# mycophonic/saprobe-alac

Measured on AMD Instinct MI355X. Metric: Msamples/s decoded (16-bit stereo, 4096-frame packets), higher is better.
Workload: dtype int32; 1 GPU; 65536 packets/GPU x 16-bit 2-ch 4096-frame ALAC, music-like synthetic, device-resident in/out; packets_per_gpu=65536

## Files before the change

### saprobe-alac_amd/csrc/alac_duo.h

```cpp
#ifndef ALAC_DUO_H
#define ALAC_DUO_H

#include <type_traits>

#include "alac_regular.h"

namespace alac {

constexpr uint32_t DUO_CHUNK = 16;
constexpr int DUO_UN8_MAX = 12;
enum { ROLE_A = 0, ROLE_B = 1, ROLE_BOTH = 2, ROLE_C = 3 };

template <class W, class B, int NA, int OUT, int ROLE, bool F16, bool NARROW, bool EA, bool UN8W = false, bool EC = false, int WMODE = 0>
ALAC_DEV void duo_phase(W& wv, const DevCfg& cfg, const B& bits, RegLane<W>& s, uint32_t size, uint32_t ns,
                        uint32_t n_it, uint32_t hdr_pos, uint32_t den_shift, uint32_t chan_bits, int32_t mix_res,
                        uint32_t mix_sh, uint32_t na_rt, uint32_t shift_pos, uint32_t sb, uint32_t mode) {
    constexpr bool DO_A = ROLE == ROLE_A || ROLE == ROLE_BOTH, DO_B = ROLE == ROLE_B || ROLE == ROLE_BOTH;
    constexpr bool RAW = OUT == OUT_RAW;
    constexpr bool LAST = OUT == OUT_STEREO || OUT == OUT_MONO || RAW;
    constexpr bool CPE = OUT == OUT_STEREO;
    constexpr bool QND = W::kResMem || EC;
    constexpr bool GEN = NA == 0;
    constexpr int NR = GEN ? 1 : NA;
    constexpr bool WRAP = !(NA == 4 || NA == 5 || NA == 6 || NA == 8);
// ... 54 lines not shown
    const uint32_t nzm = mix_res != 0 ? 0xffffffffu : 0u;

    uint32_t ns_live = s.err == 0 ? ns : 0u;
    if (DO_A) gol_head(s, c31kb);
    auto qval = [&](uint32_t nd) -> int32_t { return QND ? (int32_t)nd : gol_unfold(nd); };
    auto golomb_chunk = [&](uint32_t c) {
        const uint32_t buf = c & 1u;
        if ((c + 1u) * CH <= n_it) {
#pragma nounroll
            for (uint32_t g = 0; g < CH; g += GOL_TICK) {
                s.rd.tick(wv, s.pos);
                s.near = gol_near(s, c * CH + g, ns_live);
#pragma nounroll
                for (uint32_t h = g; h < g + GOL_TICK; h += 4u) {
#pragma unroll
                    for (uint32_t j = 0; j < 4u; ++j)
                        wv.rq_write(buf, h + j, qval(gol_step<true>(wv, bits, s, size, kb, wb, c31kb, chan_bits, c * CH + h + j, ns, ns_live)));
                }
            }
            return;
        }
#pragma nounroll
        for (uint32_t j = 0; j < CH; ++j) {
            const uint32_t i = c * CH + j;
            if (i >= n_it) break;
            if ((i & (GOL_TICK - 1u)) == 0) {
                s.rd.tick(wv, s.pos);
                s.near = gol_near(s, i, ns_live);
            }
            wv.rq_write(buf, j, qval(gol_step<true>(wv, bits, s, size, kb, wb, c31kb, chan_bits, i, ns, ns_live)));
        }
    };
    constexpr bool FP_OK = F16 && CPE && LAST && !EMIT_A && !RAW;
    uint32_t fp_base = 0, fp_inc = 0;
    using fp_yes = std::integral_constant<bool, true>;
    using fp_no = std::integral_constant<bool, false>;
    auto emit = [&](uint32_t i, int32_t o, int32_t u, uint64_t sw, uint32_t jj, auto fp) {
        constexpr bool FP = decltype(fp)::value;
        const bool on = i < ns;
        if (RAW) {
            wv.st_push_if((uint32_t)o, on);
            return;
        }
        int32_t l = o, r = 0;
        if (CPE) {
            const int32_t vv = o;
            const int32_t mv = NARROW ? ALAC_MUL24(mix_res, vv) : (int32_t)((uint32_t)mix_res * (uint32_t)vv);
            l = u + (int32_t)((uint32_t)vv & nzm) - (mv >> mix_sh);
            r = (int32_t)((((uint32_t)(l - vv)) & nzm) | ((uint32_t)vv & ~nzm));
        }
        if (F16) {
            const uint32_t pcm = ((uint32_t)l & 0xffffu) | ((uint32_t)r << 16);
            if (FP) wv.st_put(fp_base, jj, pcm, fp_inc);
            else wv.st_push_if(pcm, on);
            return;
        }
        if (cfg.bit_depth == 20) {
            l = (int32_t)((uint32_t)l << 4);
            r = (int32_t)((uint32_t)r << 4);
        }
        if (merge_any) {
            const uint32_t sh_l = sb ? (uint32_t)(sw >> (64u - sb)) : 0u;
            const uint32_t sh_r = (CPE && sb) ? (uint32_t)((sw << sb) >> (64u - sb)) : 0u;
            l = (int32_t)((uint32_t)l << sb) | (int32_t)sh_l;
            r = (int32_t)((uint32_t)r << sb) | (int32_t)sh_r;
        }
// ... 97 lines not shown
    uint64_t sw_n[CH];
    uint32_t g_n[CH / 4u][3] = {};
    auto fetch_mem_ahead = [&](uint32_t c) {
        const bool blocks = whole_pk3(c);
#pragma unroll
        for (uint32_t j = 0; j < CH; ++j) {
            const uint32_t i = c * CH + j;
            u_n[j] = 0;
            sw_n[j] = 0;
            if (i < n_it) {
                if (CPE) u_n[j] = *wv.u_row(i);
                if (merge_any && !blocks) sw_n[j] = bits.window_raw(shift_pos + i * sstep_a);
            }
        }
        if (PK3C && blocks && sb8) {
#pragma unroll
            for (uint32_t q = 0; q < CH / 4u; ++q) bits.load12(sh_byte + 2u * (c * CH + 4u * q), g_n[q][0], g_n[q][1], g_n[q][2]);
        }
    };
    auto emit_chunk = [&](uint32_t c) {
        if (PK3C && whole_pk3(c)) {
#pragma unroll
            for (uint32_t q = 0; q < CH / 4u; ++q) {
                int32_t vv4[4], uu4[4];
#pragma unroll
                for (uint32_t j = 0; j < 4u; ++j) {
                    vv4[j] = sq_v[4u * q + j];
                    uu4[j] = u_v[4u * q + j];
                }
                pk3_block(c * CH + 4u * q, vv4, uu4, g_v[q][0], g_v[q][1], g_v[q][2]);
            }
            return;
        }
#pragma unroll
        for (uint32_t j = 0; j < CH; ++j) {
            const uint32_t i = c * CH + j;
            if (i < n_it) emit(i, sq_v[j], u_v[j], sw_v[j], 0u, fp_no{});
        }
        wv.st_step();
    };
    constexpr uint32_t UN = (NARROW && (((F16 || !LAST || RAW || EMIT_A) && NR <= DUO_UN8_MAX) || (UN8W && NR <= 8))) ? 8u : 4u;
    constexpr bool HBM_IN = LAST && !RAW && !EMIT_A;
    constexpr bool RMEM = W::kResMem && ROLE == ROLE_B;
    int32_t dpre[UN];
    uint32_t dpre_row = 0xffffffffu;
    int32_t upre[UN];
    uint64_t spre[UN];
    uint32_t pre_row = 0xffffffffu;
    constexpr uint32_t NSUB = UN / 4u;
    uint32_t gpre[NSUB][3] = {};
    auto prefetch_group = [&](uint32_t row0) {
        pre_row = row0;
#pragma unroll
        for (uint32_t j = 0; j < UN; ++j) {
            upre[j] = 0;
            spre[j] = 0;
            if (CPE) upre[j] = *wv.u_row(row0 + j);
            if (merge_any && !pk3) spre[j] = bits.window_raw(shift_pos + (row0 + j) * sstep_b);
        }
        if (PK3 && pk3 && sb8) {
#pragma unroll
            for (uint32_t q = 0; q < NSUB; ++q) bits.load12(sh_byte + 2u * (row0 + 4u * q), gpre[q][0], gpre[q][1], gpre[q][2]);
        }
    };
    auto predict_chunk = [&](uint32_t c) {
        const uint32_t buf = c & 1u;
        const bool simple = GEN && (na == 0 || na == 31);
        const uint32_t sstep = (CPE ? 2u : 1u) * sb;
        if (!simple && !mode_any && c * CH > na && (c + 1u) * CH <= n_it) {
            auto groups = [&](auto wrap, auto fp) {
                constexpr bool FP = decltype(fp)::value;
#pragma nounroll
// ... 456 lines not shown
```

### saprobe-alac_amd/csrc/alac_gpu.h

```cpp
#ifndef ALAC_GPU_H
#define ALAC_GPU_H
#include <hip/hip_runtime.h>

#include <algorithm>
#include <cstdio>
#include <cstdlib>
#include <cstring>

#define ALAC_DEV __device__ __forceinline__
#define ALAC_HD __host__ __device__ __forceinline__
#define ALAC_NOINLINE
#define ALAC_MUL24(a, b) __mul24((int)(a), (int)(b))
__device__ __forceinline__ uint32_t alac_sad(uint32_t a, uint32_t b, uint32_t c) {
    uint32_t r;
    asm("v_sad_u32 %0, %1, %2, %3" : "=v"(r) : "v"(a), "v"(b), "v"(c));
    return r;
}
#define ALAC_SAD(a, b, c) alac_sad((uint32_t)(a), (uint32_t)(b), (uint32_t)(c))

__device__ __forceinline__ int32_t alac_sign_med3(int32_t x) {
    int32_t r;
    asm("v_med3_i32 %0, %1, -1, 1" : "=v"(r) : "v"(x));
    return r;
}
// ... 104 lines not shown
#ifndef ALAC_LDS_ROWS
#define ALAC_LDS_ROWS 64
#endif
#ifndef ALAC_LDS_RING
#define ALAC_LDS_RING 32
#endif
#ifndef ALAC_LDS_FLUSH
#define ALAC_LDS_FLUSH (ALAC_LDS_ROWS / 2)
#endif
constexpr uint32_t kRing = ALAC_LDS_ROWS;
constexpr uint32_t kFlush = ALAC_LDS_FLUSH;
static_assert(kFlush <= kRing && kRing % 4 == 0 && (kFlush == 16 || kFlush == 32), "the stager flushes 64- or 128-byte pieces of its rows");
constexpr uint32_t kRowStride = kRing + 1;
constexpr uint32_t kFallbackSlots = 64;
constexpr uint32_t kRingDw = ALAC_LDS_RING;
constexpr uint32_t kRingSlots = kRingDw + 2;

constexpr uint32_t kKeys = alac::KEY_IRREGULAR + 2u;
constexpr uint32_t kKeyLegacy = alac::KEY_IRREGULAR;
constexpr uint32_t kKeyScan = alac::KEY_IRREGULAR + 1u;
struct Plan {
    uint32_t count[kKeys];
    uint32_t pkt_start[kKeys];
    uint32_t cursor[kKeys];
    uint32_t nk;
    uint32_t list_key[kKeys];
    uint32_t list_wave0[kKeys];
    uint32_t total_waves;
    uint32_t irr_waves;
    uint32_t wide_waves;
    uint32_t gate[2][512];
    uint32_t balance[2][512];
    uint32_t queue[2];
};

static __shared__ uint32_t s_rows[kWave * kRowStride];
static __shared__ unsigned long long s_optr[kWave];
static __shared__ __attribute__((aligned(16))) uint32_t s_ring[kRingSlots * kWave];
constexpr uint32_t kQ = alac::DUO_CHUNK;
static __shared__ int32_t s_rq[2 * kQ * kWave];

__host__ __device__ inline size_t u_tile_cells(uint32_t frame_length) { return ((size_t)frame_length + 1u) * kWave; }

struct GpuWave {
    static constexpr bool kResMem = false;
    static constexpr uint32_t kRingDw = alack::kRingDw;
    int32_t* u_tile;
    int32_t* g_tile;
    uint8_t* my_out;
    uint32_t lane, wcnt, flushed;
    uint32_t ppw;

    ALAC_DEV bool any(bool p) const { return __ballot(p) != 0ull; }
    ALAC_DEV uint32_t max_u32(uint32_t v) const {
#pragma unroll
        for (int o = 32; o > 0; o >>= 1) {
            const uint32_t t = (uint32_t)__shfl_xor((int)v, o, 64);
            v = t > v ? t : v;
        }
        return (uint32_t)__builtin_amdgcn_readfirstlane((int)v);
    }
    static constexpr bool kRingPow2 = (kRing & (kRing - 1u)) == 0u;
    uint32_t wpos, fpos;
    ALAC_DEV static uint32_t umin_(uint32_t a, uint32_t b) { return a < b ? a : b; }
    ALAC_DEV static uint32_t st_wrap(uint32_t x) { return kRingPow2 ? (x & (kRing - 1u)) : umin_(x, x - kRing); }
    ALAC_DEV uint32_t st_pos() const { return kRingPow2 ? (wcnt & (kRing - 1u)) : wpos; }
// ... 121 lines not shown
    }
    ALAC_DEV uint32_t quad_from_below(uint32_t x, uint32_t fresh, uint32_t q0m) const {
        return ALAC_BFI(q0m, fresh, (uint32_t)__builtin_amdgcn_mov_dpp((int)x, 0x90, 0xf, 0xf, true));
    }
    ALAC_DEV void duo_sync() { asm volatile("s_waitcnt lgkmcnt(0)\n\ts_barrier" ::: "memory"); }
    ALAC_DEV void duo_sync_mem() {
        __threadfence_block();
        __syncthreads();
    }
    ALAC_DEV int32_t* u_row(uint32_t i) const { return u_tile + ((size_t)i * kWave + (ppw < kWave ? (lane < ppw ? lane : ppw) : lane)); }
    ALAC_DEV int32_t* g_slot(uint32_t k) const { return g_tile + (size_t)k * ppw; }
};

struct GpuWaveMem : GpuWave {
    static constexpr bool kResMem = true;
    const int32_t* res;
    uint32_t it, chunk0;
    ALAC_DEV int32_t rq_read(uint32_t, uint32_t j) const { return res[chunk0 + j]; }
    ALAC_DEV void rq_write(uint32_t, uint32_t, int32_t) {}
    ALAC_DEV void duo_sync() {
        ++it;
        chunk0 = (it - 1u) * kQ;
    }
    ALAC_DEV void duo_sync_mem() {}
};

__device__ __forceinline__ uint32_t avail_of(uint64_t blob_bytes, uint64_t off) {
    const uint64_t left = blob_bytes - off;
    return left > 0xffffffffull ? 0xffffffffu : (uint32_t)left;
}

__global__ void alac_classify(alac::DevCfg cfg, const uint8_t* __restrict__ blob, uint64_t blob_bytes, const uint64_t* __restrict__ offsets,
                              const uint32_t* __restrict__ sizes, uint32_t n, uint16_t* __restrict__ keys, uint32_t* __restrict__ sizes_ws,
                              uint32_t* __restrict__ frames_out, int32_t* __restrict__ status, Plan* plan);
__global__ void alac_plan(Plan* plan, uint32_t ppw);
__global__ void alac_cu_census(uint32_t* __restrict__ seen, uint32_t* __restrict__ arrived, uint32_t expect);
__global__ void alac_scatter(const uint16_t* __restrict__ keys, uint32_t n, Plan* plan, uint32_t* __restrict__ perm);
__global__ void alac_task_classify(alac::DevCfg cfg, const alac::ChanDesc* __restrict__ cd, const alac::PktDesc* __restrict__ pd,
                                   const uint16_t* __restrict__ pkt_keys, uint32_t n_slots, uint16_t* __restrict__ keys, Plan* plan);
__global__ void alac_scan(alac::DevCfg cfg, const uint8_t* __restrict__ blob, uint64_t blob_bytes, const uint64_t* __restrict__ offsets,
                          const uint32_t* __restrict__ sizes, const uint32_t* __restrict__ perm, const Plan* __restrict__ plan,
                          uint8_t* __restrict__ out, uint64_t out_stride, uint32_t* __restrict__ frames_out,
                          int32_t* __restrict__ status, int32_t* __restrict__ scratch_u, int32_t* __restrict__ scratch_g,
                          uint32_t ppw, alac::ChanDesc* __restrict__ cd, alac::PktDesc* __restrict__ pd, int32_t* __restrict__ rows,
                          uint64_t row_stride);
__global__ void alac_legacy(alac::DevCfg cfg, const uint8_t* __restrict__ blob, uint64_t blob_bytes, const uint64_t* __restrict__ offsets,
                            const uint32_t* __restrict__ sizes, const uint32_t* __restrict__ perm, const Plan* __restrict__ plan,
                            const alac::PktDesc* __restrict__ pd, uint8_t* __restrict__ out, uint64_t out_stride,
                            uint32_t* __restrict__ frames_out, int32_t* __restrict__ status, int32_t* __restrict__ scratch_u,
                            int32_t* __restrict__ scratch_g, uint32_t ppw);
constexpr uint32_t kModeFit4 = 4u, kModeFit5 = 5u, kModeGated = 6u;
constexpr __host__ __device__ __forceinline__ uint32_t decode_mode(uint32_t items, uint32_t n_cu, uint32_t cap, uint32_t force, bool mono,
                                                                  bool fit5) {
    if (force == kModeFit4 || (force == kModeFit5 && fit5)) return force;
    if (items <= 4u * n_cu) return kModeFit4;
    if (items <= 5u * n_cu) return (cap >= 5u && !mono) ? kModeGated : fit5 ? kModeFit5 : kModeFit4;
    if (items <= 6u * n_cu && cap >= 6u) return kModeGated;
    return (2u * items <= 15u * n_cu || !fit5) ? kModeFit4 : kModeFit5;
}
constexpr __host__ __device__ __forceinline__ uint32_t pair_quota(uint32_t items, uint32_t n_cu, uint32_t cap) {
    const uint32_t need = (items + n_cu - 1u) / n_cu;
    return need < 5u ? 5u : need < cap ? need : cap;
}
constexpr bool mode_is_fit4_without_the_others(uint32_t n_cu) {
    for (uint32_t items = 0u; items <= 40u * n_cu; items += (items < 8u * n_cu ? 1u : n_cu / 2u + 1u))
        if (decode_mode(items, n_cu, 0u, 0u, false, false) != kModeFit4 || decode_mode(items, n_cu, 0u, 5u, true, false) != kModeFit4) return false;
    return true;
}
constexpr bool mode_is_fit4_within_four(uint32_t n_cu) {
    for (uint32_t cap = 0u; cap <= 8u; ++cap)
// ... 52 lines not shown
```

### saprobe-alac_amd/csrc/alacgpu.hip

```cpp
#include "alac_gpu.h"
#include "alac_host.h"
#include "alac_waveform.h"

using namespace alack;

namespace {
thread_local char g_err[512] = "";
}

void alack::set_err(const char* fmt, ...) {
    va_list ap;
    va_start(ap, fmt);
    vsnprintf(g_err, sizeof(g_err), fmt, ap);
    va_end(ap);
}

namespace {

class CopyPool {
public:
    explicit CopyPool(unsigned threads) {
        for (unsigned t = 0; t < threads; ++t) workers_.emplace_back([this] { run(); });
    }
    ~CopyPool() {
// ... 97 lines not shown
Kernels choose_kernels(const alac::DevCfg& c) {
    Kernels k{};
    k.lean = alac::lean_config(c);
    k.one_or_two = c.num_channels <= 2;
    k.quad = c.bit_depth == 16 ? ALAC_PAIR_KERNEL(alac_decode_16q) : c.bit_depth == 32 ? ALAC_PAIR_KERNEL(alac_decode_32q) : ALAC_PAIR_KERNEL(alac_decode_24q);
    k.gated = c.bit_depth == 16 ? ALAC_PAIR_KERNEL(alac_decode_16g) : PairKernel{nullptr, ""};
    k.wide = c.bit_depth == 32 ? ALAC_PAIR_KERNEL(alac_decode_w32) : c.bit_depth == 24 ? ALAC_PAIR_KERNEL(alac_decode_w24) : PairKernel{nullptr, ""};
    const bool four_frames = c.num_channels > 2 && (c.num_channels * c.bps) % 4u == 0u;
    k.interleave = four_frames ? alac_interleave4 : alac_interleave;
    k.interleave_lds = (four_frames ? 128u : 32u) * kWave;
    k.irregular = !k.lean        ? "alac_scan (whole-packet decoder)"
                  : k.one_or_two ? "alac_scan + alac_interleave (+ alac_legacy)"
                  : four_frames  ? "alac_scan + alac_chan_predict + alac_interleave4 (+ alac_legacy)"
                                 : "alac_scan + alac_chan_predict + alac_interleave (+ alac_legacy)";
    return k;
}
#undef ALAC_PAIR_KERNEL

}

struct alacgpu_decoder {
    alacgpu_config cfg;
    alac::DevCfg dev_cfg;
    Kernels kernels;
    int device;
    size_t frame_bytes;
    hipStream_t stream;
    hipStream_t s_in, s_out;
    hipStream_t s_side;
    hipEvent_t ev_fork, ev_join;
    hipEvent_t ev_start[kTimingSlots], ev_stop[kTimingSlots];
    uint64_t launches;
    DevBuf scratch_u, scratch_g, plan, cls, perm, sizes_ws;
    DevBuf cd, pd, plan2, keys2, perm2, rows;
    Slot slots[kSlots];
    CopyPool* pool;
    uint32_t n_cu;
    DevBuf cu_number;
    size_t chunk_bytes;
    uint32_t lanes_min;
    int side;
    std::thread* ahead;
    int ahead_rc;
    char ahead_err[512];
    size_t last_n;
    uint32_t last_ppw, last_cap, last_fit5;
    uint32_t fit_force;
    DevBuf wave_ws;
    hipEvent_t ev_w0, ev_w1;
    bool wave_timed;
};

namespace {

size_t plan_claims_offset() { return (sizeof(Plan) + 255u) & ~(size_t)255u; }
size_t plan_bytes(size_t waves) { return plan_claims_offset() + waves * 4 * sizeof(uint32_t); }

struct KernelAttr {
    uint32_t pairs_per_cu, static_lds;
};
KernelAttr kernel_attr(void (*kernel)(PairArgs)) {
    static std::mutex mu;
    static std::vector<std::pair<const void*, KernelAttr>> cache;
    std::lock_guard<std::mutex> g(mu);
    for (const auto& e : cache)
        if (e.first == (const void*)kernel) return e.second;
    int v = 0;
    hipFuncAttributes at;
    KernelAttr a{4u, kQuadLdsFit4};
    if (hipOccupancyMaxActiveBlocksPerMultiprocessor(&v, kernel, (int)(2 * kWave), 0) == hipSuccess && v > 0) a.pairs_per_cu = (uint32_t)v;
    else (void)hipGetLastError();
    if (hipFuncGetAttributes(&at, (const void*)kernel) == hipSuccess) a.static_lds = (uint32_t)at.sharedSizeBytes;
    else (void)hipGetLastError();
    cache.emplace_back((const void*)kernel, a);
    return a;
}

int cu_numbers(alacgpu_decoder* dec) {
    int rc;
    if ((rc = dec->cu_number.ensure(513 * sizeof(uint32_t)))) return rc;
    HIP_TRY(hipMemsetAsync(dec->cu_number.p, 0, 513 * sizeof(uint32_t), dec->stream));
    hipLaunchKernelGGL(alac_cu_census, dim3(2 * dec->n_cu), dim3(kWave), 0, dec->stream, (uint32_t*)dec->cu_number.p,
                       (uint32_t*)dec->cu_number.p + 512, 2 * dec->n_cu);
    HIP_TRY(hipGetLastError());
    uint32_t seen[512];
    HIP_TRY(hipMemcpyAsync(seen, dec->cu_number.p, sizeof(seen), hipMemcpyDeviceToHost, dec->stream));
    HIP_TRY(hipStreamSynchronize(dec->stream));
    uint32_t per_xcd[8] = {0}, xcds = 0, total = 0;
    for (uint32_t i = 0; i < 512; i++)
// ... 10 lines not shown
        if (seen[i]) {
            const uint32_t x = i >> 6;
            seen[i] = 1u + next[x]++ * xcds + order[x];
        }
    if (total > dec->n_cu) dec->n_cu = total;
    HIP_TRY(hipMemcpyAsync(dec->cu_number.p, seen, sizeof(seen), hipMemcpyHostToDevice, dec->stream));
    HIP_TRY(hipStreamSynchronize(dec->stream));
    return ALACGPU_E_OK;
}

size_t max_waves(uint32_t bit_depth, size_t n, uint32_t ppw) {
    const size_t keys = (bit_depth >= 24 ? 2 : 1) * 18 * 18 + 8;
    return (n + ppw - 1) / ppw + std::min<size_t>(n, keys);
}
size_t max_waves(const alacgpu_decoder* dec, size_t n, uint32_t ppw) { return max_waves(dec->cfg.bit_depth, n, ppw); }

uint32_t pick_ppw(size_t n) {
    if (const char* e = getenv("ALACGPU_PPW")) {
        const int v = atoi(e);
        if (v >= 1 && v <= 64) return (uint32_t)v;
    }
    uint32_t ppw = kWave;
    while (ppw > 1 && n / ppw < 256) ppw >>= 1;
    return ppw;
}

size_t row_stride_of(uint32_t frame_length) { return ((size_t)frame_length + 3u) & ~(size_t)3u; }

int reserve_workspace(alacgpu_decoder* dec, size_t n, uint32_t ppw) {
    const size_t waves = max_waves(dec, n, ppw);
    int rc;
    if ((rc = dec->scratch_u.ensure(waves * u_tile_cells(dec->cfg.frame_length) * sizeof(int32_t)))) return rc;
    if ((rc = dec->scratch_g.ensure(waves * kFallbackSlots * ppw * sizeof(int32_t)))) return rc;
    if ((rc = dec->plan.ensure(plan_bytes(waves)))) return rc;
    if ((rc = dec->cls.ensure((n ? n : 1) * sizeof(uint16_t)))) return rc;
    if ((rc = dec->perm.ensure((n ? n : 1) * sizeof(uint32_t)))) return rc;
    if ((rc = dec->sizes_ws.ensure((n ? n : 1) * sizeof(uint32_t)))) return rc;
    const size_t ns = (n ? n : 1) * 8;
    if ((rc = dec->cd.ensure(ns * sizeof(alac::ChanDesc)))) return rc;
    if ((rc = dec->pd.ensure((n ? n : 1) * sizeof(alac::PktDesc)))) return rc;
    if (dec->cfg.num_channels > 2) {
        if ((rc = dec->plan2.ensure(sizeof(Plan)))) return rc;
        if ((rc = dec->keys2.ensure(ns * sizeof(uint16_t)))) return rc;
        if ((rc = dec->perm2.ensure(ns * sizeof(uint32_t)))) return rc;
        if ((rc = dec->rows.ensure((n ? n : 1) * dec->cfg.num_channels * row_stride_of(dec->cfg.frame_length) * sizeof(int32_t))))
            return rc;
    }
    return ALACGPU_E_OK;
}

struct Launch {
    alacgpu_decoder* dec;
    alac::DevCfg c;
    const uint8_t* d_blob;
    uint64_t blob_bytes;
    const uint64_t* d_offsets;
    size_t n;
    uint8_t* d_out;
    size_t out_stride;
    uint32_t* d_frames;
    int32_t* d_status;
    uint32_t ppw;
    size_t waves;
    hipStream_t irr;
    bool forked;
    uint32_t scan_grid;
    Plan* plan() const { return (Plan*)dec->plan.p; }
    const uint32_t* sz() const { return (const uint32_t*)dec->sizes_ws.p; }
};

struct SideFork {
    alacgpu_decoder* dec;
    bool open = false;
    int fork() {
        HIP_TRY(hipEventRecord(dec->ev_fork, dec->stream));
        HIP_TRY(hipStreamWaitEvent(dec->s_side, dec->ev_fork, 0));
        open = true;
        return ALACGPU_E_OK;
    }
    int join() {
        HIP_TRY(hipEventRecord(dec->ev_join, dec->s_side));
        HIP_TRY(hipStreamWaitEvent(dec->stream, dec->ev_join, 0));
        open = false;
        return ALACGPU_E_OK;
    }
    ~SideFork() {
        if (open) (void)hipStreamSynchronize(dec->s_side);
    }
};

int sort_pass(const Launch& L, const uint32_t* d_sizes) {
    alacgpu_decoder* dec = L.dec;
    const uint32_t nb = (uint32_t)((L.n + 255) / 256);
    HIP_TRY(hipMemsetAsync(L.plan(), 0, plan_bytes(L.waves), dec->stream));
    hipLaunchKernelGGL(alac_classify, dim3(nb), dim3(256), 0, dec->stream, L.c, L.d_blob, L.blob_bytes, L.d_offsets, d_sizes,
                       (uint32_t)L.n, (uint16_t*)dec->cls.p, (uint32_t*)dec->sizes_ws.p, L.d_frames, L.d_status, L.plan());
    hipLaunchKernelGGL(alac_plan, dim3(1), dim3(kWave), 0, dec->stream, L.plan(), L.ppw);
    hipLaunchKernelGGL(alac_scatter, dim3(nb), dim3(256), 0, dec->stream, (const uint16_t*)dec->cls.p, (uint32_t)L.n, L.plan(),
                       (uint32_t*)dec->perm.p);
    return ALACGPU_E_OK;
}

void scan(const Launch& L) {
    alacgpu_decoder* dec = L.dec;
    hipLaunchKernelGGL(alac_scan, dim3(L.scan_grid), dim3(kWave), 0, L.irr, L.c, L.d_blob, L.blob_bytes,
                       L.d_offsets, L.sz(), (const uint32_t*)dec->perm.p, (const Plan*)L.plan(), L.d_out, (uint64_t)L.out_stride, L.d_frames,
                       L.d_status, (int32_t*)dec->scratch_u.p, (int32_t*)dec->scratch_g.p, L.ppw, (alac::ChanDesc*)dec->cd.p,
                       (alac::PktDesc*)dec->pd.p, dec->cfg.num_channels > 2 ? (int32_t*)dec->rows.p : (int32_t*)nullptr,
                       (uint64_t)row_stride_of(dec->cfg.frame_length));
}

void narrow_launch(const Launch& L, const PairArgs& a, uint32_t slots, uint32_t mode) {
    alacgpu_decoder* dec = L.dec;
    const Kernels& k = dec->kernels;
    if (mode == kModeGated) {
        if (a.cap) hipLaunchKernelGGL(k.gated.fn, dim3(std::min<uint32_t>(a.cap * dec->n_cu, slots)), dim3(2 * kWave), 0, dec->stream, a);
        return;
    }
    if (mode == kModeFit5 && !a.fit5) return;
    const uint32_t stat = kernel_attr(k.quad.fn).static_lds;
    PairArgs q = a;
    q.fit = mode;
    hipLaunchKernelGGL(k.quad.fn, dim3(slots), dim3(4 * kWave), (mode == kModeFit4 && stat < kQuadLdsFit4) ? kQuadLdsFit4 - stat : 0u,
                       dec->stream, q);
}

void regular_packets(const Launch& L) {
    alacgpu_decoder* dec = L.dec;
    const Kernels& k = dec->kernels;
    const size_t n = L.n;
    const uint32_t ppw = L.ppw;
    PairArgs a{L.c, L.d_blob, (uint64_t)L.blob_bytes, L.d_offsets, L.sz(), (const uint32_t*)dec->perm.p, L.plan(), L.d_out, (uint64_t)L.out_stride,
               L.d_frames, L.d_status, (int32_t*)dec->scratch_u.p, (const uint32_t*)dec->cu_number.p,
               (uint32_t*)((uint8_t*)L.plan() + plan_claims_offset()), ppw, dec->n_cu, 0u, dec->lanes_min, 4u, dec->fit_force, 0u};
    const uint32_t slots = (uint32_t)L.waves;
    const uint32_t n_cu = dec->n_cu;
    const bool beyond4 = (n + ppw - 1) / ppw > (size_t)4 * n_cu || dec->fit_force == kModeFit5;
    const bool has_twin = k.gated.fn && beyond4 && dec->fit_force == 0u;
    {
        const uint32_t stat = kernel_attr(k.quad.fn).static_lds;
        a.fit5 = (beyond4 && (size_t)((stat + 1279u) / 1280u) * 1280u * 5u <= 163840u) ? 1u : 0u;
    }
    if (has_twin) a.cap = kernel_attr(k.gated.fn).pairs_per_cu;
    if (a.cap <= 4u) a.cap = 0u;
    dec->last_cap = a.cap;
    dec->last_fit5 = a.fit5;
    const uint32_t guess = decode_mode((uint32_t)((n + ppw - 1) / ppw), n_cu, a.cap, dec->fit_force, dec->cfg.num_channels == 1, a.fit5 != 0u);
    narrow_launch(L, a, slots, guess);
    if (k.wide.fn) hipLaunchKernelGGL(k.wide.fn, dim3(slots), dim3(2 * kWave), 0, dec->stream, a);
    for (uint32_t mode : {kModeFit4, kModeFit5, kModeGated})
        if (mode != guess) narrow_launch(L, a, slots, mode);
}

int split_pipeline(const Launch& L) {
    alacgpu_decoder* dec = L.dec;
    Plan* plan2 = (Plan*)dec->plan2.p;
    const size_t n_slots = L.n * 8;
    const uint32_t nb2 = (uint32_t)((n_slots + 255) / 256);
    const uint32_t ppw2 = pick_ppw(L.n * dec->cfg.num_channels);
    HIP_TRY(hipMemsetAsync(plan2, 0, sizeof(Plan), dec->stream));
    hipLaunchKernelGGL(alac_task_classify, dim3(nb2), dim3(256), 0, dec->stream, L.c, (const alac::ChanDesc*)dec->cd.p,
                       (const alac::PktDesc*)dec->pd.p, (const uint16_t*)dec->cls.p, (uint32_t)n_slots,
                       (uint16_t*)dec->keys2.p, plan2);
    hipLaunchKernelGGL(alac_plan, dim3(1), dim3(kWave), 0, dec->stream, plan2, ppw2);
    hipLaunchKernelGGL(alac_scatter, dim3(nb2), dim3(256), 0, dec->stream, (const uint16_t*)dec->keys2.p,
                       (uint32_t)n_slots, plan2, (uint32_t*)dec->perm2.p);
    hipLaunchKernelGGL(alac_chan_predict, dim3((uint32_t)max_waves(16u, n_slots, ppw2)), dim3(kWave), 0, dec->stream, L.c,
                       L.d_blob, L.blob_bytes, L.d_offsets, L.sz(), (const uint32_t*)dec->perm2.p, (const Plan*)plan2,
                       (const alac::ChanDesc*)dec->cd.p, (int32_t*)dec->rows.p, (uint64_t)row_stride_of(dec->cfg.frame_length), ppw2);
    return ALACGPU_E_OK;
}

void irregular_pcm(const Launch& L) {
    alacgpu_decoder* dec = L.dec;
    const Kernels& k = dec->kernels;
    const uint64_t rs = row_stride_of(dec->cfg.frame_length);
    const uint32_t bpp = (dec->cfg.frame_length + kWave - 1u) / kWave;
    const uint32_t ib = (uint32_t)std::min<uint64_t>((uint64_t)L.n * ((bpp + 7u) / 8u), L.forked ? (uint64_t)4 * dec->n_cu : (uint64_t)32768u);
    hipLaunchKernelGGL(k.interleave, dim3(ib), dim3(kWave), k.interleave_lds, L.irr, L.c, L.d_blob, L.blob_bytes, L.d_offsets, L.sz(),
                       (const uint32_t*)dec->perm.p, (const Plan*)L.plan(), (const alac::ChanDesc*)dec->cd.p,
                       (const alac::PktDesc*)dec->pd.p, (const int32_t*)dec->rows.p, rs, L.d_out, (uint64_t)L.out_stride, bpp);
    hipLaunchKernelGGL(alac_legacy, dim3(L.scan_grid), dim3(kWave), 0, L.irr, L.c, L.d_blob, L.blob_bytes,
                       L.d_offsets, L.sz(), (const uint32_t*)dec->perm.p, (const Plan*)L.plan(), (const alac::PktDesc*)dec->pd.p, L.d_out,
                       (uint64_t)L.out_stride, L.d_frames, L.d_status, (int32_t*)dec->scratch_u.p, (int32_t*)dec->scratch_g.p, L.ppw);
}

int launch(alacgpu_decoder* dec, const uint8_t* d_blob, uint64_t blob_bytes, const uint64_t* d_offsets,
           const uint32_t* d_sizes, size_t n, uint8_t* d_out, size_t out_stride, uint32_t* d_frames, int32_t* d_status) {
    if (n == 0) return ALACGPU_E_OK;
    if (n > 0x7fffffffu) {
        set_err("batch too large");
        return ALACGPU_E_ARG;
    }
    const uint32_t ppw = pick_ppw(n);
    int rc = reserve_workspace(dec, n, ppw);
    if (rc) return rc;
    dec->last_n = n;
    dec->last_ppw = ppw;
    dec->last_cap = dec->last_fit5 = 0;
// ... 516 lines not shown
        return ALACGPU_E_DECODE;
    }
    *out_len = (size_t)frames * d->cfg.num_channels * (size_t)d->dev_cfg.bps;
    return ALACGPU_E_OK;
}

int alacgpu_timing_reset(alacgpu_decoder* d) {
    if (!d) return ALACGPU_E_ARG;
    d->launches = 0;
    return ALACGPU_E_OK;
}

int alacgpu_kernel_times(alacgpu_decoder* d, float* ms, size_t max_n, size_t* n_out) {
    if (!d || !ms || !n_out) return ALACGPU_E_ARG;
    HIP_TRY(hipSetDevice(d->device));
    HIP_TRY(hipStreamSynchronize(d->stream));
    size_t avail = (size_t)std::min<uint64_t>(d->launches, kTimingSlots);
    size_t n = std::min(avail, max_n);
    for (size_t i = 0; i < n; i++) {
        const uint32_t slot = (uint32_t)((d->launches - n + i) % kTimingSlots);
        HIP_TRY(hipEventElapsedTime(&ms[i], d->ev_start[slot], d->ev_stop[slot]));
    }
    *n_out = n;
    return ALACGPU_E_OK;
}

int alacgpu_pair_placement(alacgpu_decoder* d, uint32_t* tags, size_t max_n, size_t* n_out) {
    if (!d || !tags || !n_out) return ALACGPU_E_ARG;
    HIP_TRY(hipSetDevice(d->device));
    HIP_TRY(hipStreamSynchronize(d->stream));
    *n_out = 0;
    if (!d->plan.p) return ALACGPU_E_OK;
    Plan head;
    HIP_TRY(hipMemcpy(&head, d->plan.p, sizeof(Plan), hipMemcpyDeviceToHost));
    const size_t n = std::min<size_t>(head.total_waves, max_n / 4);
    if (plan_bytes(n) > d->plan.cap) return ALACGPU_E_ARG;
    if (n) HIP_TRY(hipMemcpy(tags, (const uint8_t*)d->plan.p + plan_claims_offset(), n * 4 * sizeof(uint32_t), hipMemcpyDeviceToHost));
    *n_out = n;
    return ALACGPU_E_OK;
}

int alacgpu_last_dispatch(alacgpu_decoder* d, alacgpu_dispatch* out) {
    if (!d || !out) return ALACGPU_E_ARG;
    HIP_TRY(hipSetDevice(d->device));
    HIP_TRY(hipStreamSynchronize(d->stream));
    memset(out, 0, sizeof(*out));
    if (!d->plan.p || d->last_n == 0) return ALACGPU_E_OK;
    Plan head;
    HIP_TRY(hipMemcpy(&head, d->plan.p, sizeof(Plan), hipMemcpyDeviceToHost));
    out->packets_per_slot = d->last_ppw;
    out->slots = head.total_waves;
    out->irregular_slots = head.irr_waves;
    out->wide_slots = head.wide_waves;
    out->narrow_slots = head.total_waves - head.irr_waves - head.wide_waves;
    out->keys = head.nk;
    const Kernels& k = d->kernels;
    const bool lean = k.one_or_two && k.lean;
    const char* narrow = "";
    if (lean && out->narrow_slots) {
        const uint32_t mode = decode_mode(out->narrow_slots, d->n_cu, d->last_cap, d->fit_force, d->cfg.num_channels == 1, d->last_fit5 != 0u);
        narrow = mode == kModeGated ? k.gated.name : k.quad.name;
        out->gated = mode == kModeGated ? 1u : 0u;
        out->workgroups_per_cu = mode == kModeGated ? pair_quota(out->narrow_slots, d->n_cu, d->last_cap) : mode;
        if (!out->gated && out->narrow_slots <= d->n_cu + d->n_cu / 8u && d->lanes_min <= 16u) out->lanes_per_packet = d->last_ppw <= 32u ? 4u : 2u;
    }
    snprintf(out->narrow_kernel, sizeof(out->narrow_kernel), "%s", narrow);
    snprintf(out->wide_kernel, sizeof(out->wide_kernel), "%s", (lean && out->wide_slots) ? k.wide.name : "");
    snprintf(out->irregular_kernels, sizeof(out->irregular_kernels), "%s", out->irregular_slots ? k.irregular : "");
    return ALACGPU_E_OK;
}

int alacgpu_last_kernel_ms(alacgpu_decoder* d, float* ms) {
    size_t got = 0;
    int rc = alacgpu_kernel_times(d, ms, 1, &got);
    if (rc) return rc;
    if (got == 0) {
        set_err("no kernel has been launched on this handle since the last timing reset");
        return ALACGPU_E_ARG;
    }
    return ALACGPU_E_OK;
}

// ... 79 lines not shown
```

### saprobe-alac_amd/csrc/k_sort.hip

```cpp
#include "alac_gpu.h"

namespace alack {

__global__ void __launch_bounds__(256)
alac_classify(alac::DevCfg cfg, const uint8_t* __restrict__ blob, uint64_t blob_bytes, const uint64_t* __restrict__ offsets,
              const uint32_t* __restrict__ sizes, uint32_t n, uint16_t* __restrict__ keys, uint32_t* __restrict__ sizes_ws,
              uint32_t* __restrict__ frames_out, int32_t* __restrict__ status, Plan* plan) {
    __shared__ uint32_t hist[kKeys];
    for (uint32_t k = threadIdx.x; k < kKeys; k += blockDim.x) hist[k] = 0;
    __syncthreads();
    const uint32_t i = blockIdx.x * blockDim.x + threadIdx.x;
    if (i < n) {
        const uint64_t off = offsets[i];
        uint64_t sz = sizes ? (uint64_t)sizes[i] : offsets[i + 1] - off;
        const bool ok = off <= blob_bytes && sz <= blob_bytes - off && sz <= 0x0fffffffull &&
                        (sizes || offsets[i + 1] >= off);
        if (!ok) {
            keys[i] = (uint16_t)alac::TASK_NONE;
            sizes_ws[i] = 0;
            frames_out[i] = 0;
            status[i] = ALACGPU_ERR_RANGE;
        } else if (sz == 0) {
            keys[i] = (uint16_t)alac::TASK_NONE;
            sizes_ws[i] = 0;
            frames_out[i] = 0;
            status[i] = ALACGPU_STATUS(alac::ST_OVERRUN, 0, 0);
        } else {
            sizes_ws[i] = (uint32_t)sz;
            const uint8_t* p = blob + off;
            uint32_t key = alac::classify_regular(cfg, p, (uint32_t)sz, avail_of(blob_bytes, off));
            if (key == alac::KEY_IRREGULAR) key = alac::lean_config(cfg) ? kKeyScan : kKeyLegacy;
            keys[i] = (uint16_t)key;
            atomicAdd(&hist[key], 1u);
        }
    }
    __syncthreads();
    for (uint32_t k = threadIdx.x; k < kKeys; k += blockDim.x)
        if (hist[k]) atomicAdd(&plan->count[k], hist[k]);
}

__global__ void __launch_bounds__(kWave) alac_plan(Plan* plan, uint32_t ppw) {
    __shared__ uint32_t cnt[kKeys];
    for (uint32_t k = threadIdx.x; k < kKeys; k += kWave) cnt[k] = plan->count[k];
    __syncthreads();
    constexpr uint32_t R = (kKeys + kWave - 1) / kWave;
    const uint32_t q0 = threadIdx.x * R;
    uint32_t p = 0, w = 0, z = 0, wi = 0, ww = 0;
    for (uint32_t r = 0; r < R; ++r) {
        const uint32_t q = q0 + r;
        if (q >= kKeys) break;
        const uint32_t key = kKeys - 1u - q;
        const uint32_t c = cnt[key];
        const uint32_t cw = (c + ppw - 1) / ppw;
        p += c;
        w += cw;
        z += c ? 1u : 0u;
        wi += key >= alac::KEY_IRREGULAR ? cw : 0u;
        ww += (key >= alac::KEY_WIDE && key < alac::KEY_IRREGULAR) ? cw : 0u;
    }
    uint32_t ip = p, iw = w, iz = z, ii = wi, ix = ww;
#pragma unroll
    for (int o = 1; o < (int)kWave; o <<= 1) {
        const uint32_t tp = (uint32_t)__shfl_up((int)ip, o, kWave), tw = (uint32_t)__shfl_up((int)iw, o, kWave);
        const uint32_t tz = (uint32_t)__shfl_up((int)iz, o, kWave), ti = (uint32_t)__shfl_up((int)ii, o, kWave);
        const uint32_t tx = (uint32_t)__shfl_up((int)ix, o, kWave);
        if ((int)threadIdx.x >= o) {
            ix += tx;
            ip += tp;
            iw += tw;
            iz += tz;
            ii += ti;
        }
    }
    uint32_t ep = ip - p, ew = iw - w, ez = iz - z;
    for (uint32_t r = 0; r < R; ++r) {
        const uint32_t q = q0 + r;
        if (q >= kKeys) break;
        const uint32_t key = kKeys - 1u - q;
        const uint32_t c = cnt[key];
        plan->pkt_start[key] = ep;
        plan->cursor[key] = 0;
        if (c) {
            plan->list_key[ez] = key;
            plan->list_wave0[ez] = ew;
            ++ez;
            ep += c;
            ew += (c + ppw - 1) / ppw;
        }
    }
    if (threadIdx.x == kWave - 1u) {
        plan->nk = iz;
        plan->total_waves = iw;
        plan->irr_waves = ii;
        plan->wide_waves = ix;
    }
}

__global__ void __launch_bounds__(256)
alac_scatter(const uint16_t* __restrict__ keys, uint32_t n, Plan* plan, uint32_t* __restrict__ perm) {
    __shared__ uint32_t hist[kKeys];
    __shared__ uint32_t base[kKeys];
    for (uint32_t k = threadIdx.x; k < kKeys; k += blockDim.x) hist[k] = 0;
    __syncthreads();
    const uint32_t i = blockIdx.x * blockDim.x + threadIdx.x;
    uint32_t key = 0, local = 0;
    if (i < n) {
        key = keys[i];
        if (key != alac::TASK_NONE) local = atomicAdd(&hist[key], 1u);
    }
    __syncthreads();
    for (uint32_t k = threadIdx.x; k < kKeys; k += blockDim.x)
        if (hist[k]) base[k] = plan->pkt_start[k] + atomicAdd(&plan->cursor[k], hist[k]);
    __syncthreads();
    if (i < n && key != alac::TASK_NONE) perm[base[key] + local] = i;
}

__global__ void __launch_bounds__(256)
alac_task_classify(alac::DevCfg cfg, const alac::ChanDesc* __restrict__ cd, const alac::PktDesc* __restrict__ pd,
                   const uint16_t* __restrict__ pkt_keys, uint32_t n_slots, uint16_t* __restrict__ keys, Plan* plan) {
    __shared__ uint32_t hist[alac::NUM_TASK_KEYS];
    if (threadIdx.x < alac::NUM_TASK_KEYS) hist[threadIdx.x] = 0;
    __syncthreads();
    const uint32_t t = blockIdx.x * blockDim.x + threadIdx.x;
    if (t < n_slots) {
        const uint32_t pkt = t >> 3, slot = t & 7u;
        uint32_t key = alac::TASK_NONE;
        if (pkt_keys[pkt] == kKeyScan) {
            const alac::PktDesc q = pd[pkt];
            if (q.status == 0 && q.route == alac::ROUTE_SPLIT && slot < q.nslots) {
                const alac::ChanDesc d = cd[t];
                if ((d.info & alac::CD_VALID) && !(d.info & alac::CD_ESCAPE)) key = alac::chan_task_key(cfg, d);
            }
        }
        keys[t] = (uint16_t)key;
// ... 23 lines not shown
```

Measured before the change: 256,700 Msamples/s.

## Fuse plan build into classify via last-block ticket and double-buffer plan wipe

Removes the separate memset and single-wave alac_plan launch from the sort pass. The last classify block, chosen by an atomic ticket, builds the plan with a 256-thread multi-wave scan. The plan buffer is double-buffered, and the stale half is zeroed inside the scatter kernel. A fast-path emit for the EC/EMIT_A chunk route is also added. This trades two launches for a grid-wide atomic and fence sequence, and it depends on correct memory ordering between blocks.

```diff
diff --git a/saprobe-alac_amd/csrc/alac_duo.h b/saprobe-alac_amd/csrc/alac_duo.h
--- a/saprobe-alac_amd/csrc/alac_duo.h
+++ b/saprobe-alac_amd/csrc/alac_duo.h
@@ -110,6 +110,7 @@
         }
     };
     constexpr bool FP_OK = F16 && CPE && LAST && !EMIT_A && !RAW;
+    constexpr bool FP_C = F16 && CPE && EMIT_A && EC && DO_C;
     uint32_t fp_base = 0, fp_inc = 0;
     using fp_yes = std::integral_constant<bool, true>;
     using fp_no = std::integral_constant<bool, false>;
@@ -273,12 +274,24 @@
             }
             return;
         }
+        const bool whole_fp = FP_C && (c + 1u) * CH <= n_it;
+        const bool ends_here = whole_fp && ns > c * CH && ns < (c + 1u) * CH;
+        if (FP_C && whole_fp && !wv.any(ends_here)) {
+            fp_inc = ns >= (c + 1u) * CH ? CH : 0u;
+            fp_base = wv.st_group_base(CH);
+#pragma unroll
+            for (uint32_t j = 0; j < CH; ++j) emit(c * CH + j, sq_v[j], u_v[j], sw_v[j], j, fp_yes{});
+            wv.st_advance(fp_inc);
+            wv.st_step();
+            return;
+        }
 #pragma unroll
         for (uint32_t j = 0; j < CH; ++j) {
             const uint32_t i = c * CH + j;
             if (i < n_it) emit(i, sq_v[j], u_v[j], sw_v[j], 0u, fp_no{});
         }
         wv.st_step();
+        if (FP_C && ends_here) (void)wv.st_finish();
     };
     constexpr uint32_t UN = (NARROW && (((F16 || !LAST || RAW || EMIT_A) && NR <= DUO_UN8_MAX) || (UN8W && NR <= 8))) ? 8u : 4u;
     constexpr bool HBM_IN = LAST && !RAW && !EMIT_A;
diff --git a/saprobe-alac_amd/csrc/alac_gpu.h b/saprobe-alac_amd/csrc/alac_gpu.h
--- a/saprobe-alac_amd/csrc/alac_gpu.h
+++ b/saprobe-alac_amd/csrc/alac_gpu.h
@@ -160,6 +160,7 @@
     uint32_t gate[2][512];
     uint32_t balance[2][512];
     uint32_t queue[2];
+    uint32_t ticket;
 };
 
 static __shared__ uint32_t s_rows[kWave * kRowStride];
@@ -347,10 +348,11 @@
 
 __global__ void alac_classify(alac::DevCfg cfg, const uint8_t* __restrict__ blob, uint64_t blob_bytes, const uint64_t* __restrict__ offsets,
                               const uint32_t* __restrict__ sizes, uint32_t n, uint16_t* __restrict__ keys, uint32_t* __restrict__ sizes_ws,
-                              uint32_t* __restrict__ frames_out, int32_t* __restrict__ status, Plan* plan);
+                              uint32_t* __restrict__ frames_out, int32_t* __restrict__ status, Plan* plan, uint32_t ppw);
 __global__ void alac_plan(Plan* plan, uint32_t ppw);
 __global__ void alac_cu_census(uint32_t* __restrict__ seen, uint32_t* __restrict__ arrived, uint32_t expect);
-__global__ void alac_scatter(const uint16_t* __restrict__ keys, uint32_t n, Plan* plan, uint32_t* __restrict__ perm);
+__global__ void alac_scatter(const uint16_t* __restrict__ keys, uint32_t n, Plan* plan, uint32_t* __restrict__ perm, uint4* __restrict__ wipe,
+                             uint32_t wipe_n);
 __global__ void alac_task_classify(alac::DevCfg cfg, const alac::ChanDesc* __restrict__ cd, const alac::PktDesc* __restrict__ pd,
                                    const uint16_t* __restrict__ pkt_keys, uint32_t n_slots, uint16_t* __restrict__ keys, Plan* plan);
 __global__ void alac_scan(alac::DevCfg cfg, const uint8_t* __restrict__ blob, uint64_t blob_bytes, const uint64_t* __restrict__ offsets,
diff --git a/saprobe-alac_amd/csrc/alacgpu.hip b/saprobe-alac_amd/csrc/alacgpu.hip
--- a/saprobe-alac_amd/csrc/alacgpu.hip
+++ b/saprobe-alac_amd/csrc/alacgpu.hip
@@ -153,6 +153,8 @@
     hipEvent_t ev_start[kTimingSlots], ev_stop[kTimingSlots];
     uint64_t launches;
     DevBuf scratch_u, scratch_g, plan, cls, perm, sizes_ws;
+    size_t plan_half, plan_dirty;
+    uint32_t plan_cur;
     DevBuf cd, pd, plan2, keys2, perm2, rows;
     Slot slots[kSlots];
     CopyPool* pool;
@@ -176,6 +178,7 @@
 
 size_t plan_claims_offset() { return (sizeof(Plan) + 255u) & ~(size_t)255u; }
 size_t plan_bytes(size_t waves) { return plan_claims_offset() + waves * 4 * sizeof(uint32_t); }
+uint8_t* plan_now(const alacgpu_decoder* dec) { return (uint8_t*)dec->plan.p + dec->plan_cur * dec->plan_half; }
 
 struct KernelAttr {
     uint32_t pairs_per_cu, static_lds;
@@ -252,7 +255,14 @@
     int rc;
     if ((rc = dec->scratch_u.ensure(waves * u_tile_cells(dec->cfg.frame_length) * sizeof(int32_t)))) return rc;
     if ((rc = dec->scratch_g.ensure(waves * kFallbackSlots * ppw * sizeof(int32_t)))) return rc;
-    if ((rc = dec->plan.ensure(plan_bytes(waves)))) return rc;
+    const size_t both = 2 * ((plan_bytes(waves) + 255u) & ~(size_t)255u);
+    if (both > dec->plan.cap) {
+        if ((rc = dec->plan.ensure(both))) return rc;
+        dec->plan_half = (dec->plan.cap / 2) & ~(size_t)255u;
+        dec->plan_dirty = 0;
+        dec->plan_cur = 0;
+        HIP_TRY(hipMemsetAsync(dec->plan.p, 0, dec->plan.cap, dec->stream));
+    }
     if ((rc = dec->cls.ensure((n ? n : 1) * sizeof(uint16_t)))) return rc;
     if ((rc = dec->perm.ensure((n ? n : 1) * sizeof(uint32_t)))) return rc;
     if ((rc = dec->sizes_ws.ensure((n ? n : 1) * sizeof(uint32_t)))) return rc;
@@ -285,7 +295,7 @@
     hipStream_t irr;
     bool forked;
     uint32_t scan_grid;
-    Plan* plan() const { return (Plan*)dec->plan.p; }
+    Plan* plan() const { return (Plan*)plan_now(dec); }
     const uint32_t* sz() const { return (const uint32_t*)dec->sizes_ws.p; }
 };
 
@@ -312,12 +322,14 @@
 int sort_pass(const Launch& L, const uint32_t* d_sizes) {
     alacgpu_decoder* dec = L.dec;
     const uint32_t nb = (uint32_t)((L.n + 255) / 256);
-    HIP_TRY(hipMemsetAsync(L.plan(), 0, plan_bytes(L.waves), dec->stream));
+    uint4* const wipe = (uint4*)plan_now(dec);
+    const uint32_t wipe_n = (uint32_t)(dec->plan_dirty / sizeof(uint4));
+    dec->plan_cur ^= 1u;
+    dec->plan_dirty = plan_bytes(L.waves);
     hipLaunchKernelGGL(alac_classify, dim3(nb), dim3(256), 0, dec->stream, L.c, L.d_blob, L.blob_bytes, L.d_offsets, d_sizes,
-                       (uint32_t)L.n, (uint16_t*)dec->cls.p, (uint32_t*)dec->sizes_ws.p, L.d_frames, L.d_status, L.plan());
-    hipLaunchKernelGGL(alac_plan, dim3(1), dim3(kWave), 0, dec->stream, L.plan(), L.ppw);
+                       (uint32_t)L.n, (uint16_t*)dec->cls.p, (uint32_t*)dec->sizes_ws.p, L.d_frames, L.d_status, L.plan(), L.ppw);
     hipLaunchKernelGGL(alac_scatter, dim3(nb), dim3(256), 0, dec->stream, (const uint16_t*)dec->cls.p, (uint32_t)L.n, L.plan(),
-                       (uint32_t*)dec->perm.p);
+                       (uint32_t*)dec->perm.p, wipe, wipe_n);
     return ALACGPU_E_OK;
 }
 
@@ -382,9 +394,9 @@
     hipLaunchKernelGGL(alac_task_classify, dim3(nb2), dim3(256), 0, dec->stream, L.c, (const alac::ChanDesc*)dec->cd.p,
                        (const alac::PktDesc*)dec->pd.p, (const uint16_t*)dec->cls.p, (uint32_t)n_slots,
                        (uint16_t*)dec->keys2.p, plan2);
-    hipLaunchKernelGGL(alac_plan, dim3(1), dim3(kWave), 0, dec->stream, plan2, ppw2);
+    hipLaunchKernelGGL(alac_plan, dim3(1), dim3(256), 0, dec->stream, plan2, ppw2);
     hipLaunchKernelGGL(alac_scatter, dim3(nb2), dim3(256), 0, dec->stream, (const uint16_t*)dec->keys2.p,
-                       (uint32_t)n_slots, plan2, (uint32_t*)dec->perm2.p);
+                       (uint32_t)n_slots, plan2, (uint32_t*)dec->perm2.p, (uint4*)nullptr, 0u);
     hipLaunchKernelGGL(alac_chan_predict, dim3((uint32_t)max_waves(16u, n_slots, ppw2)), dim3(kWave), 0, dec->stream, L.c,
                        L.d_blob, L.blob_bytes, L.d_offsets, L.sz(), (const uint32_t*)dec->perm2.p, (const Plan*)plan2,
                        (const alac::ChanDesc*)dec->cd.p, (int32_t*)dec->rows.p, (uint64_t)row_stride_of(dec->cfg.frame_length), ppw2);
@@ -967,10 +979,10 @@
     *n_out = 0;
     if (!d->plan.p) return ALACGPU_E_OK;
     Plan head;
-    HIP_TRY(hipMemcpy(&head, d->plan.p, sizeof(Plan), hipMemcpyDeviceToHost));
+    HIP_TRY(hipMemcpy(&head, plan_now(d), sizeof(Plan), hipMemcpyDeviceToHost));
     const size_t n = std::min<size_t>(head.total_waves, max_n / 4);
-    if (plan_bytes(n) > d->plan.cap) return ALACGPU_E_ARG;
-    if (n) HIP_TRY(hipMemcpy(tags, (const uint8_t*)d->plan.p + plan_claims_offset(), n * 4 * sizeof(uint32_t), hipMemcpyDeviceToHost));
+    if (plan_bytes(n) > d->plan_half) return ALACGPU_E_ARG;
+    if (n) HIP_TRY(hipMemcpy(tags, plan_now(d) + plan_claims_offset(), n * 4 * sizeof(uint32_t), hipMemcpyDeviceToHost));
     *n_out = n;
     return ALACGPU_E_OK;
 }
@@ -982,7 +994,7 @@
     memset(out, 0, sizeof(*out));
     if (!d->plan.p || d->last_n == 0) return ALACGPU_E_OK;
     Plan head;
-    HIP_TRY(hipMemcpy(&head, d->plan.p, sizeof(Plan), hipMemcpyDeviceToHost));
+    HIP_TRY(hipMemcpy(&head, plan_now(d), sizeof(Plan), hipMemcpyDeviceToHost));
     out->packets_per_slot = d->last_ppw;
     out->slots = head.total_waves;
     out->irregular_slots = head.irr_waves;
diff --git a/saprobe-alac_amd/csrc/k_sort.hip b/saprobe-alac_amd/csrc/k_sort.hip
--- a/saprobe-alac_amd/csrc/k_sort.hip
+++ b/saprobe-alac_amd/csrc/k_sort.hip
@@ -2,11 +2,83 @@
 
 namespace alack {
 
+template <uint32_t NT>
+__device__ __forceinline__ void plan_build(Plan* plan, uint32_t ppw, uint32_t* cnt , uint32_t* part ) {
+    constexpr uint32_t NW = NT / kWave;
+    constexpr uint32_t R = (kKeys + NT - 1) / NT;
+    for (uint32_t k = threadIdx.x; k < kKeys; k += NT) cnt[k] = __hip_atomic_load(&plan->count[k], __ATOMIC_RELAXED, __HIP_MEMORY_SCOPE_AGENT);
+    __syncthreads();
+    const uint32_t q0 = threadIdx.x * R;
+    uint32_t v[5] = {0, 0, 0, 0, 0};
+    for (uint32_t r = 0; r < R; ++r) {
+        const uint32_t q = q0 + r;
+        if (q >= kKeys) break;
+        const uint32_t key = kKeys - 1u - q;
+        const uint32_t c = cnt[key];
+        const uint32_t cw = (c + ppw - 1) / ppw;
+        v[0] += c;
+        v[1] += cw;
+        v[2] += c ? 1u : 0u;
+        v[3] += key >= alac::KEY_IRREGULAR ? cw : 0u;
+        v[4] += (key >= alac::KEY_WIDE && key < alac::KEY_IRREGULAR) ? cw : 0u;
+    }
+    const uint32_t lane = threadIdx.x % kWave, wave = threadIdx.x / kWave;
+    uint32_t inc[5];
+#pragma unroll
+    for (int j = 0; j < 5; ++j) {
+        uint32_t x = v[j];
+#pragma unroll
+        for (int o = 1; o < (int)kWave; o <<= 1) {
+            const uint32_t t = (uint32_t)__shfl_up((int)x, o, kWave);
+            if ((int)lane >= o) x += t;
+        }
+        inc[j] = x;
+        if (lane == kWave - 1u) part[j * NW + wave] = x;
+    }
+    __syncthreads();
+#pragma unroll
+    for (int j = 0; j < 5; ++j)
+        for (uint32_t w = 0; w < wave; ++w) inc[j] += part[j * NW + w];
+    uint32_t ep = inc[0] - v[0], ew = inc[1] - v[1], ez = inc[2] - v[2];
+    for (uint32_t r = 0; r < R; ++r) {
+        const uint32_t q = q0 + r;
+        if (q >= kKeys) break;
+        const uint32_t key = kKeys - 1u - q;
+        const uint32_t c = cnt[key];
+        plan->pkt_start[key] = ep;
+        if (c) {
+            plan->list_key[ez] = key;
+            plan->list_wave0[ez] = ew;
+            ++ez;
+            ep += c;
+            ew += (c + ppw - 1) / ppw;
+        }
+    }
+    if (threadIdx.x == NT - 1u) {
+        plan->nk = inc[2];
+        plan->total_waves = inc[1];
+        plan->irr_waves = inc[3];
+        plan->wide_waves = inc[4];
+    }
+}
+
+template <uint32_t NT>
+__device__ __forceinline__ void plan_by_last(Plan* plan, uint32_t ppw, uint32_t* cnt, uint32_t* part) {
+    asm volatile("s_waitcnt vmcnt(0)" ::: "memory");
+    __syncthreads();
+    if (threadIdx.x == 0) part[0] = __hip_atomic_fetch_add(&plan->ticket, 1u, __ATOMIC_RELAXED, __HIP_MEMORY_SCOPE_AGENT);
+    __syncthreads();
+    const bool last = part[0] == gridDim.x - 1u;
+    __syncthreads();
+    if (last) plan_build<NT>(plan, ppw, cnt, part);
+}
+
 __global__ void __launch_bounds__(256)
 alac_classify(alac::DevCfg cfg, const uint8_t* __restrict__ blob, uint64_t blob_bytes, const uint64_t* __restrict__ offsets,
               const uint32_t* __restrict__ sizes, uint32_t n, uint16_t* __restrict__ keys, uint32_t* __restrict__ sizes_ws,
-              uint32_t* __restrict__ frames_out, int32_t* __restrict__ status, Plan* plan) {
+              uint32_t* __restrict__ frames_out, int32_t* __restrict__ status, Plan* plan, uint32_t ppw) {
     __shared__ uint32_t hist[kKeys];
+    __shared__ uint32_t part[5 * 256 / kWave];
     for (uint32_t k = threadIdx.x; k < kKeys; k += blockDim.x) hist[k] = 0;
     __syncthreads();
     const uint32_t i = blockIdx.x * blockDim.x + threadIdx.x;
@@ -36,70 +108,22 @@
     }
     __syncthreads();
     for (uint32_t k = threadIdx.x; k < kKeys; k += blockDim.x)
-        if (hist[k]) atomicAdd(&plan->count[k], hist[k]);
+        if (hist[k]) __hip_atomic_fetch_add(&plan->count[k], hist[k], __ATOMIC_RELAXED, __HIP_MEMORY_SCOPE_AGENT);
+    plan_by_last<256>(plan, ppw, hist, part);
 }
 
-__global__ void __launch_bounds__(kWave) alac_plan(Plan* plan, uint32_t ppw) {
+__global__ void __launch_bounds__(256) alac_plan(Plan* plan, uint32_t ppw) {
     __shared__ uint32_t cnt[kKeys];
-    for (uint32_t k = threadIdx.x; k < kKeys; k += kWave) cnt[k] = plan->count[k];
-    __syncthreads();
-    constexpr uint32_t R = (kKeys + kWave - 1) / kWave;
-    const uint32_t q0 = threadIdx.x * R;
-    uint32_t p = 0, w = 0, z = 0, wi = 0, ww = 0;
-    for (uint32_t r = 0; r < R; ++r) {
-        const uint32_t q = q0 + r;
-        if (q >= kKeys) break;
-        const uint32_t key = kKeys - 1u - q;
-        const uint32_t c = cnt[key];
-        const uint32_t cw = (c + ppw - 1) / ppw;
-        p += c;
-        w += cw;
-        z += c ? 1u : 0u;
-        wi += key >= alac::KEY_IRREGULAR ? cw : 0u;
-        ww += (key >= alac::KEY_WIDE && key < alac::KEY_IRREGULAR) ? cw : 0u;
-    }
-    uint32_t ip = p, iw = w, iz = z, ii = wi, ix = ww;
-#pragma unroll
-    for (int o = 1; o < (int)kWave; o <<= 1) {
-        const uint32_t tp = (uint32_t)__shfl_up((int)ip, o, kWave), tw = (uint32_t)__shfl_up((int)iw, o, kWave);
-        const uint32_t tz = (uint32_t)__shfl_up((int)iz, o, kWave), ti = (uint32_t)__shfl_up((int)ii, o, kWave);
-        const uint32_t tx = (uint32_t)__shfl_up((int)ix, o, kWave);
-        if ((int)threadIdx.x >= o) {
-            ix += tx;
-            ip += tp;
-            iw += tw;
-            iz += tz;
-            ii += ti;
-        }
-    }
-    uint32_t ep = ip - p, ew = iw - w, ez = iz - z;
-    for (uint32_t r = 0; r < R; ++r) {
-        const uint32_t q = q0 + r;
-        if (q >= kKeys) break;
-        const uint32_t key = kKeys - 1u - q;
-        const uint32_t c = cnt[key];
-        plan->pkt_start[key] = ep;
-        plan->cursor[key] = 0;
-        if (c) {
-            plan->list_key[ez] = key;
-            plan->list_wave0[ez] = ew;
-            ++ez;
-            ep += c;
-            ew += (c + ppw - 1) / ppw;
-        }
-    }
-    if (threadIdx.x == kWave - 1u) {
-        plan->nk = iz;
-        plan->total_waves = iw;
-        plan->irr_waves = ii;
-        plan->wide_waves = ix;
-    }
+    __shared__ uint32_t part[5 * 256 / kWave];
+    plan_build<256>(plan, ppw, cnt, part);
 }
 
 __global__ void __launch_bounds__(256)
-alac_scatter(const uint16_t* __restrict__ keys, uint32_t n, Plan* plan, uint32_t* __restrict__ perm) {
+alac_scatter(const uint16_t* __restrict__ keys, uint32_t n, Plan* plan, uint32_t* __restrict__ perm, uint4* __restrict__ wipe,
+             uint32_t wipe_n) {
     __shared__ uint32_t hist[kKeys];
     __shared__ uint32_t base[kKeys];
+    for (uint32_t w = blockIdx.x * blockDim.x + threadIdx.x; w < wipe_n; w += gridDim.x * blockDim.x) wipe[w] = make_uint4(0u, 0u, 0u, 0u);
     for (uint32_t k = threadIdx.x; k < kKeys; k += blockDim.x) hist[k] = 0;
     __syncthreads();
     const uint32_t i = blockIdx.x * blockDim.x + threadIdx.x;
```

After: 258,200 Msamples/s (median of 6 runs). Within noise of the previous version (+0.6%).
